# biotite-dev/springcraft

Measured on AMD Instinct MI355X. Metric: ANM modes/sec (Hessian build + full eigensolve), N=2000 C-alpha, higher is better.
Workload: dtype f64; 1 GPU; C3: N=2000 C-alpha ANM, HinsenForceField (no cutoff), full 6000x6000 eigensolve, all modes + vectors; parallelism=independent structures sharded over GPUs, no data-path collective

## Files before the change

### springcraft_amd/csrc/eigh_internal.h

```cpp
#pragma once

#include "common.h"
#include "gemm_f64.h"

struct TriLayout {
  int n, nb;
  long long slab;
  long long vw;
  long long wv;
  long long xraw;
  long long ypart;
  long long dpart;
  long long npart;
  long long wvpart;
  long long d, e, tau;
  long long hscale;
  long long rctl;
  long long rrec;
};
inline size_t tri_resident_bytes(int n) { return sizeof(double) * (8 + (size_t)6 * ((n + 63) / 64 * 64)); }

int mirror_lower_batched(sc_ctx* ctx, double* d_a, long long stride_a, int n, int batch);
int prepare_matrix_batched(sc_ctx* ctx, double* d_a, long long stride_a, int n, int batch, double* d_tri_ws,
                           const TriLayout& L);
int unscale_values_batched(sc_ctx* ctx, double* d_w, long long stride_w, int m, int batch, const double* d_tri_ws,
                           const TriLayout& L);

int tridiag_batched(sc_ctx* ctx, double* d_a, long long stride_a, int n, int batch, double* d_ws,
                    const TriLayout& L, const GemmDesc* d_syr2k_descs, float* ms_symv, float* ms_syr2k);
bool resident_enabled(const sc_ctx* ctx);

struct DcNode {
  int lo, mid, hi;
};

struct DcLayout {
  int n;
  int leaf_max;
  long long slab;
  long long dd, ee;
  long long w0, w1;
  long long z;
  long long dl, zz;
  long long ddef;
  long long lam;
  long long tauv;
  long long zhat;
  long long rot_c, rot_s;
  long long scale;
  long long src;
  long long org;
  long long dest;
  long long rot_a, rot_b;
  long long ktop_src, ktop_k;
  long long kbot_src, kbot_k;
  long long cnt;
};

int stedc_batched(sc_ctx* ctx, int n, int batch, const double* d_tri_ws, const TriLayout& TL,
                  double* d_dc_ws, const DcLayout& DL, double* d_w, long long stride_w,
                  double* d_q_out, double* d_q_tmp, double* d_u, long long stride_q,
                  GemmDesc* d_merge_descs );
size_t dc_slab_doubles(int n, DcLayout* out);
int dc_max_nodes(int n, int leaf_max);

int sturm_bisect_batched(sc_ctx* ctx, int n, int batch, const double* d_tri_ws, const TriLayout& TL,
                         double* d_w, long long stride_w);

struct BtLayout {
  int n, nbt, splits;
  long long slab;
  long long vc;
  long long gram;
  long long t;
  long long g12;
  long long tx;
  long long w1;
  long long w2;
  int splits_g;
};
size_t bt_slab_doubles(int n, BtLayout* out);
int bt_desc_count(int n, int batch);
int backtransform_batched(sc_ctx* ctx, double* d_a, long long stride_a, int n, int batch,
                          const double* d_tri_ws, const TriLayout& TL, double* d_bt_ws,
                          const BtLayout& BL, double* d_z, long long stride_z, int ncols, double* d_vt,
                          GemmDesc* d_descs , int off = 1, int phase = 0);

struct SbLayout {
  int n;
  long long slab;
  long long vw, wv;
  long long xv;
  long long qrpart, qrpiv;
  long long qrpart8;
  long long xsplit;
  int symm_split;
  long long small;
  long long cmat;
  long long small2;
  long long p2;
  long long ab;
  int ngroups;
  long long ndia;
  long long vd;
  long long frag;
  long long tau2;
};
size_t sb_slab_doubles(int n, int batch, SbLayout* out);
int sb_desc_count(int n, int batch);
int sb_band_width();
int sytrd_2stage_batched(sc_ctx* ctx, double* d_a, long long stride_a, int n, int batch, double* d_tri_ws,
                         const TriLayout& TL, double* d_sb_ws, const SbLayout& SL, int* d_dia_off ,
                         GemmDesc* d_descs , float* ms_stage1, float* ms_stage2,
                         double* d_band_copy = nullptr);
int bt2_prepare(sc_ctx* ctx, int n, int batch, double* d_sb_ws, const SbLayout& SL, hipStream_t st);
int bt2_batched(sc_ctx* ctx, int n, int batch, double* d_sb_ws, const SbLayout& SL, const int* d_dia_off, double* d_z,
                long long stride_z, int ncols, float* ms_fused = nullptr);

struct WinCount {
  int il, count, start, pad;
};
size_t stein_workspace_doubles(int n, int m);
int stein_batched(sc_ctx* ctx, int n, int batch, const double* d_tri_ws, const TriLayout& TL, int il, int iu,
                  double* d_w, long long stride_w, double* d_x, long long stride_x, double* d_ws,
                  GemmDesc* d_descs , const WinCount* d_win = nullptr);
int window_count_batched(sc_ctx* ctx, int batch, const double* d_tri_ws, const TriLayout& TL, double vl, double vu, int K,
                         WinCount* d_win, long long* d_count, const RaggedRec* d_own = nullptr);
int window_compact_batched(sc_ctx* ctx, int n, int batch, int K, const WinCount* d_win, double* d_w, double* d_v,
                           double* d_w_copy, double* d_v_copy);

int launch_mode_weights(sc_ctx* ctx, const double* d_w, int64_t nvec, int64_t batch, const sc_mode_selection& sel,
                        int64_t nsel, const int64_t* d_counts, double* d_s, const RaggedView* rv);
int msf_chunk(int64_t nsel);
```

### springcraft_amd/csrc/stedc.hip

```cpp
#include <algorithm>
#include <vector>

#include "eigh_internal.h"

namespace {

constexpr double kEps = 2.220446049250313e-16;

__device__ __forceinline__ int* iptr(double* ws, long long off) { return reinterpret_cast<int*>(ws + off); }
__device__ __forceinline__ const int* iptr(const double* ws, long long off) {
  return reinterpret_cast<const int*>(ws + off);
}

__device__ __forceinline__ double wave_sum_all(double v) {
#pragma unroll
  for (int off = 32; off > 0; off >>= 1) v += __shfl_xor(v, off);
  return v;
}
__device__ __forceinline__ double wave_prod_all(double v) {
#pragma unroll
  for (int off = 32; off > 0; off >>= 1) v *= __shfl_xor(v, off);
  return v;
}
__device__ __forceinline__ double wave_max_all(double v) {
#pragma unroll
  for (int off = 32; off > 0; off >>= 1) v = fmax(v, __shfl_xor(v, off));
  return v;
}

__global__ void k_dc_prepare(const double* __restrict__ tri_all, TriLayout TL, double* __restrict__ dc_all,
                             DcLayout DL, const DcNode* __restrict__ nodes, int n_nodes) {
  __shared__ double red[16];
  const double* tri = tri_all + (size_t)blockIdx.x * TL.slab;
  double* ws = dc_all + (size_t)blockIdx.x * DL.slab;
  const int n = DL.n, tid = threadIdx.x;
  double mx = 0.0;
  for (int i = tid; i < n; i += blockDim.x) {
    mx = fmax(mx, fabs(tri[TL.d + i]));
    if (i < n - 1) mx = fmax(mx, fabs(tri[TL.e + i]));
  }
  mx = wave_max_all(mx);
  if ((tid & 63) == 0) red[tid >> 6] = mx;
  __syncthreads();
  mx = 0.0;
  for (int w = 0; w < (int)(blockDim.x >> 6); ++w) mx = fmax(mx, red[w]);
  const double nrm = (mx > 0.0 && mx == mx) ? mx : 1.0;
  const double inv = 1.0 / nrm;
  for (int i = tid; i < n; i += blockDim.x) {
    const double dv = tri[TL.d + i] * inv;
    const double ev = (i < n - 1) ? tri[TL.e + i] * inv : 0.0;
    ws[DL.dd + i] = fabs(dv) < 1e-150 ? 0.0 : dv;
    ws[DL.ee + i] = fabs(ev) < 1e-150 ? 0.0 : ev;
  }
  if (tid == 0) ws[DL.scale] = nrm;
  __syncthreads();
  for (int g = tid; g < n_nodes; g += blockDim.x) {
    const int mid = nodes[g].mid;
    const double r = fabs(ws[DL.ee + mid - 1]);
    ws[DL.dd + mid - 1] -= r;
    ws[DL.dd + mid] -= r;
  }
}

template <int LEAF>
__global__ __launch_bounds__(64) void k_dc_leaves(double* __restrict__ dc_all, DcLayout DL,
                                                  const DcNode* __restrict__ leaves,
                                                  double* __restrict__ q_all, long long stride_q,
                                                  int* __restrict__ fail_flag) {
  __shared__ double Z[LEAF][LEAF + 1];
  __shared__ double d[LEAF], e[LEAF];
  double* ws = dc_all + (size_t)blockIdx.y * DL.slab;
  double* Q = q_all + (size_t)blockIdx.y * stride_q;
  const int lo = leaves[blockIdx.x].lo, hi = leaves[blockIdx.x].hi;
  const int s = hi - lo, n = DL.n;
  const int lane = threadIdx.x;
  if (lane < s) {
    for (int c = 0; c < s; ++c) Z[lane][c] = (c == lane) ? 1.0 : 0.0;
    d[lane] = ws[DL.dd + lo + lane];
    e[lane] = (lane < s - 1) ? ws[DL.ee + lo + lane] : 0.0;
  }
  __syncthreads();
  for (int l = 0; l < s; ++l) {
    int iter = 0;
    int m;
    do {
      for (m = l; m < s - 1; ++m) {
        const double dd = fabs(d[m]) + fabs(d[m + 1]);
        if (fabs(e[m]) <= kEps * dd) break;
      }
      if (m != l) {
        if (++iter > 80) {
          if (lane == 0) atomicExch(fail_flag, 1);
          break;
        }
        double g = (d[l + 1] - d[l]) / (2.0 * e[l]);
        double r = hypot(g, 1.0);
        g = d[m] - d[l] + e[l] / (g + copysign(r, g));
        double sn = 1.0, cs = 1.0, p = 0.0;
        int i;
        for (i = m - 1; i >= l; --i) {
          double f = sn * e[i];
          const double b = cs * e[i];
          r = hypot(f, g);
          __syncthreads();
          e[i + 1] = r;
          if (r == 0.0) {
            d[i + 1] -= p;
            e[m] = 0.0;
            __syncthreads();
            break;
          }
          sn = f / r;
          cs = g / r;
          g = d[i + 1] - p;
          r = (d[i] - g) * sn + 2.0 * cs * b;
          p = sn * r;
          d[i + 1] = g + p;
          g = cs * r - b;
          if (lane < s) {
            f = Z[lane][i + 1];
            Z[lane][i + 1] = sn * Z[lane][i] + cs * f;
            Z[lane][i] = cs * Z[lane][i] - sn * f;
          }
          __syncthreads();
        }
        if (r == 0.0 && i >= l) continue;
        __syncthreads();
        d[l] -= p;
        e[l] = g;
        e[m] = 0.0;
        __syncthreads();
      }
    } while (m != l);
  }
  __syncthreads();
  for (int a = 0; a < s - 1; ++a) {
    int k = a;
    double best = d[a];
    for (int b = a + 1; b < s; ++b)
      if (d[b] < best) { best = d[b]; k = b; }
    __syncthreads();
    if (k != a) {
      const double tmp = d[a];
      __syncthreads();
      d[k] = tmp;
      d[a] = best;
      if (lane < s) {
        const double t2 = Z[lane][a];
        Z[lane][a] = Z[lane][k];
        Z[lane][k] = t2;
      }
    }
    __syncthreads();
  }
  if (lane < s) {
    ws[DL.w0 + lo + lane] = d[lane];
    for (int c = 0; c < s; ++c) Q[(size_t)(lo + c) * n + lo + lane] = Z[lane][c];
  }
}

__global__ void k_dc_zero_offdiag(const DcNode* __restrict__ nodes, double* __restrict__ q_all,
                                  long long stride_q, int n) {
  const DcNode nd = nodes[blockIdx.y];
  double* Q = q_all + (size_t)blockIdx.z * stride_q;
  const int n1 = nd.mid - nd.lo, n2 = nd.hi - nd.mid;
  const long long total = 2LL * n1 * n2;
  for (long long idx = blockIdx.x * (long long)blockDim.x + threadIdx.x; idx < total;
       idx += (long long)gridDim.x * blockDim.x) {
    if (idx < (long long)n1 * n2) {
      const int r = nd.mid + (int)(idx % n2), c = nd.lo + (int)(idx / n2);
      Q[(size_t)c * n + r] = 0.0;
    } else {
      const long long k = idx - (long long)n1 * n2;
      const int r = nd.lo + (int)(k % n1), c = nd.mid + (int)(k / n1);
      Q[(size_t)c * n + r] = 0.0;
    }
  }
}

__global__ __launch_bounds__(1024) void k_dc_setup(double* __restrict__ dc_all, DcLayout DL,
                                                   const DcNode* __restrict__ nodes, int nodes_in_level,
                                                   const double* __restrict__ q_all, long long stride_q,
                                                   long long w_old_off, GemmDesc* __restrict__ descs,
                                                   int use_lds, double* __restrict__ gscratch,
                                                   long long gscratch_stride) {
  extern __shared__ __attribute__((aligned(16))) double lds[];
  __shared__ double red[16];
  __shared__ double s_tol;
  const int g = blockIdx.x, b = blockIdx.y;
  const DcNode nd = nodes[g];
  double* ws = dc_all + (size_t)b * DL.slab;
  const double* Q = q_all + (size_t)b * stride_q;
  const int n = DL.n, lo = nd.lo, mid = nd.mid, hi = nd.hi;
  const int N = hi - lo, n1 = mid - lo;
  const int tid = threadIdx.x, nthr = blockDim.x;
  const double* wold = ws + w_old_off;

  double* sd;
  double* sz;
  int* scol;
  unsigned char* smix;
  unsigned char* sflag;
  if (use_lds) {
    sd = lds;
    sz = lds + N;
    scol = reinterpret_cast<int*>(lds + 2 * N);
    smix = reinterpret_cast<unsigned char*>(scol + N);
  } else {
    double* base = gscratch + (size_t)b * gscratch_stride + 3LL * lo;
    sd = base;
    sz = base + N;
    scol = reinterpret_cast<int*>(base + 2 * N);
    smix = reinterpret_cast<unsigned char*>(scol + N);
  }
  sflag = smix + N;

  const double rho_raw = ws[DL.ee + mid - 1];
  const double sgn = rho_raw < 0.0 ? -1.0 : 1.0;
  const double rho = 2.0 * fabs(rho_raw);
  const double isq2 = 0.7071067811865475244;

  double zmax = 0.0, dmax = 0.0;
  for (int j = tid; j < N; j += nthr) {
    const int col = lo + j;
    const double zj = (j < n1 ? Q[(size_t)col * n + (mid - 1)] : sgn * Q[(size_t)col * n + mid]) * isq2;
    ws[DL.z + col] = zj;
    zmax = fmax(zmax, fabs(zj));
    dmax = fmax(dmax, fabs(wold[col]));
  }
  zmax = wave_max_all(zmax);
  dmax = wave_max_all(dmax);
  if ((tid & 63) == 0) red[tid >> 6] = fmax(zmax, dmax);
  __syncthreads();
  if (tid == 0) {
    double mx = 0.0;
    for (int w = 0; w < (nthr >> 6); ++w) mx = fmax(mx, red[w]);
    s_tol = 8.0 * kEps * mx;
  }
  __syncthreads();
  for (int j = tid; j < N; j += nthr) {
    const double v = wold[lo + j];
    int rank;
    if (j < n1) {
      int a = 0, c = N - n1;
      while (a < c) {
        const int h = (a + c) >> 1;
        if (wold[mid + h] < v) a = h + 1; else c = h;
      }
      rank = j + a;
    } else {
      int a = 0, c = n1;
      while (a < c) {
        const int h = (a + c) >> 1;
        if (wold[lo + h] <= v) a = h + 1; else c = h;
      }
      rank = (j - n1) + a;
    }
    sd[rank] = v;
    sz[rank] = ws[DL.z + lo + j];
    scol[rank] = lo + j;
    smix[rank] = 0;
  }
  __syncthreads();

  const double tol = s_tol;
  int* src = iptr(ws, DL.src);
  int* rot_a = iptr(ws, DL.rot_a);
  int* rot_b = iptr(ws, DL.rot_b);
  int* cnt = iptr(ws, DL.cnt);
  int* ktop_src = iptr(ws, DL.ktop_src);
  int* ktop_k = iptr(ws, DL.ktop_k);
  int* kbot_src = iptr(ws, DL.kbot_src);
  int* kbot_k = iptr(ws, DL.kbot_k);
  __shared__ int wsum[3][16];
  __shared__ int s_nrot;
  const int L = (N + nthr - 1) / nthr;
  const int j0 = min(tid * L, N), j1 = min(j0 + L, N);

  for (int j = tid; j < N; j += nthr) sflag[j] = !(rho * fabs(sz[j]) > tol) ? 1 : 0;
  if (tid == 0) s_nrot = 0;
  __syncthreads();
  int nseed = 0;
  for (int jj = j0; jj < j1; ++jj) {
    if (sflag[jj] & 1) continue;
    int pj = jj - 1;
    while (pj >= 0 && (sflag[pj] & 1)) --pj;
    if (pj < 0) continue;
    double s = sz[pj], c = sz[jj];
    const double tau = hypot(c, s);
    const double t = sd[jj] - sd[pj];
    c /= tau;
    s /= tau;
    if (fabs(t * c * s) <= tol) { sflag[jj] |= 2; ++nseed; }
  }
  const int any_rot = __syncthreads_or(nseed);
  if (any_rot) {
    int is = nseed;
    for (int off = 1; off < 64; off <<= 1) {
      const int us = __shfl_up(is, off);
      if ((tid & 63) >= off) is += us;
    }
    if ((tid & 63) == 63) wsum[0][tid >> 6] = is;
    __syncthreads();
    int bs = 0, total = 0;
    for (int w = 0; w < (nthr >> 6); ++w) {
      if (w < (tid >> 6)) bs += wsum[0][w];
      total += wsum[0][w];
    }
    int pos = bs + is - nseed;
    for (int jj = j0; jj < j1; ++jj)
      if (sflag[jj] & 2) kbot_k[lo + pos++] = jj;
    __syncthreads();
    if (tid == 0) {
      int nrot = 0, done_upto = -1;
      for (int si = 0; si < total; ++si) {
        int jj = kbot_k[lo + si];
        if (jj <= done_upto) continue;
        int pj = jj - 1;
        while (pj >= 0 && (sflag[pj] & 5)) --pj;
        while (true) {
          double s = sz[pj], c = sz[jj];
          const double tau = hypot(c, s);
          const double t = sd[jj] - sd[pj];
          c /= tau;
          s /= tau;
          done_upto = jj;
          if (!(fabs(t * c * s) <= tol)) break;
          sz[jj] = tau;
          sz[pj] = 0.0;
          rot_a[lo + nrot] = scol[pj];
          rot_b[lo + nrot] = scol[jj];
          ws[DL.rot_c + lo + nrot] = c;
          ws[DL.rot_s + lo + nrot] = s;
          ++nrot;
          if (((scol[pj] < mid) != (scol[jj] < mid)) || smix[pj] || smix[jj]) { smix[jj] = 1; smix[pj] = 1; }
          const double tt = sd[pj] * c * c + sd[jj] * s * s;
          sd[jj] = sd[pj] * s * s + sd[jj] * c * c;
          sd[pj] = tt;
          sflag[pj] |= 4;
          pj = jj;
          ++jj;
          while (jj < N && (sflag[jj] & 1)) ++jj;
          if (jj >= N) break;
        }
      }
      s_nrot = nrot;
    }
    __syncthreads();
  }
  {
    int ns = 0, nt = 0, nb = 0;
    for (int j = j0; j < j1; ++j)
      if (!(sflag[j] & 5)) {
        const bool top = scol[j] < mid;
        ++ns;
        nt += (top || smix[j]) ? 1 : 0;
        nb += (!top || smix[j]) ? 1 : 0;
      }
    int is = ns, it = nt, ib = nb;
    for (int off = 1; off < 64; off <<= 1) {
      const int us = __shfl_up(is, off), ut = __shfl_up(it, off), ub = __shfl_up(ib, off);
      if ((tid & 63) >= off) { is += us; it += ut; ib += ub; }
    }
    __syncthreads();
    if ((tid & 63) == 63) { wsum[0][tid >> 6] = is; wsum[1][tid >> 6] = it; wsum[2][tid >> 6] = ib; }
    __syncthreads();
    int bs = 0, bt = 0, bb = 0, ts = 0, tt = 0, tb = 0;
    for (int w = 0; w < (nthr >> 6); ++w) {
      if (w < (tid >> 6)) { bs += wsum[0][w]; bt += wsum[1][w]; bb += wsum[2][w]; }
      ts += wsum[0][w];
      tt += wsum[1][w];
      tb += wsum[2][w];
    }
    int K = bs + is - ns, K1 = bt + it - nt, K3 = bb + ib - nb;
    int ndef = j0 - K;
    for (int j = j0; j < j1; ++j) {
      if (sflag[j] & 5) {
        ws[DL.ddef + hi - 1 - ndef] = sd[j];
        src[hi - 1 - ndef] = scol[j];
        ++ndef;
      } else {
        ws[DL.dl + lo + K] = sd[j];
        ws[DL.zz + lo + K] = sz[j];
        src[lo + K] = scol[j];
        const bool top = scol[j] < mid;
        if (top || smix[j]) { ktop_src[lo + K1] = scol[j]; ktop_k[lo + K1] = K; ++K1; }
        if (!top || smix[j]) { kbot_src[lo + K3] = scol[j]; kbot_k[lo + K3] = K; ++K3; }
        ++K;
      }
    }
    if (tid == 0) {
      cnt[2 * g] = ts;
      cnt[2 * g + 1] = s_nrot;
      GemmDesc& Dt = descs[((size_t)b * nodes_in_level + g) * 2];
      Dt.n = ts;
      Dt.k = tt;
      GemmDesc& Db = descs[((size_t)b * nodes_in_level + g) * 2 + 1];
      Db.n = ts;
      Db.k = tb;
    }
  }
}

__global__ void k_dc_rotate(double* __restrict__ dc_all, DcLayout DL, const DcNode* __restrict__ nodes,
                            double* __restrict__ q_all, long long stride_q) {
  const int g = blockIdx.y, b = blockIdx.z;
  const DcNode nd = nodes[g];
  double* ws = dc_all + (size_t)b * DL.slab;
  const int nrot = iptr(ws, DL.cnt)[2 * g + 1];
  if (nrot == 0) return;
  double* Q = q_all + (size_t)b * stride_q;
  const int n = DL.n;
  const int row = nd.lo + blockIdx.x * blockDim.x + threadIdx.x;
  if (row >= nd.hi) return;
  const int* rot_a = iptr(ws, DL.rot_a) + nd.lo;
  const int* rot_b = iptr(ws, DL.rot_b) + nd.lo;
  for (int q = 0; q < nrot; ++q) {
    const double c = ws[DL.rot_c + nd.lo + q], s = ws[DL.rot_s + nd.lo + q];
    double* pa = Q + (size_t)rot_a[q] * n + row;
    double* pb = Q + (size_t)rot_b[q] * n + row;
    const double qa = *pa, qb = *pb;
    *pa = c * qa - s * qb;
    *pb = s * qa + c * qb;
  }
}

__global__ __launch_bounds__(1024) void k_dc_secular(double* __restrict__ dc_all, DcLayout DL,
                                                     const DcNode* __restrict__ nodes, int use_lds) {
  extern __shared__ __attribute__((aligned(16))) double lds[];
  const int g = blockIdx.y, b = blockIdx.z;
  const DcNode nd = nodes[g];
  double* ws = dc_all + (size_t)b * DL.slab;
  const int K = iptr(ws, DL.cnt)[2 * g];
  const int waves = blockDim.x >> 6;
  if ((int)blockIdx.x * waves >= K) return;
  const int lo = nd.lo;
  const double* dlg = ws + DL.dl + lo;
  const double* zzg = ws + DL.zz + lo;
  const double* dl;
  const double* z2;
  if (use_lds) {
    double* ldl = lds;
    double* lz2 = lds + K;
    for (int i = threadIdx.x; i < K; i += blockDim.x) {
      ldl[i] = dlg[i];
      const double z = zzg[i];
      lz2[i] = z * z;
    }
    __syncthreads();
    dl = ldl;
    z2 = lz2;
  } else {
    dl = dlg;
    z2 = nullptr;
  }
  const int lane = threadIdx.x & 63;
  const int j = blockIdx.x * waves + (threadIdx.x >> 6);
  if (j >= K) return;
  const double rho = 2.0 * fabs(ws[DL.ee + nd.mid - 1]);
  const double rinv = 1.0 / rho;

  auto fsum2 = [&](double dorg, double tau, double& fp) -> double {
    double s = 0.0, sp = 0.0;
    if (z2) {
      for (int i = lane; i < K; i += 64) {
        const double r = 1.0 / ((dl[i] - dorg) - tau);
        const double zr = z2[i] * r;
        s += zr;
        sp += zr * r;
      }
    } else {
      for (int i = lane; i < K; i += 64) {
        const double z = zzg[i];
        const double r = 1.0 / ((dl[i] - dorg) - tau);
        const double zr = z * z * r;
        s += zr;
        sp += zr * r;
      }
    }
    fp = wave_sum_all(sp);
    return rinv + wave_sum_all(s);
  };
  auto fsum = [&](double dorg, double tau) -> double {
    double fp;
    return fsum2(dorg, tau, fp);
  };

  int org;
  bool positive;
  double t_hi;
  double t_start = 0.0;
  double zj2 = 0.0, zk2 = 0.0;
  if (j == K - 1) {
    org = K - 1;
    positive = true;
    double s2 = 0.0;
    if (z2) { for (int i = lane; i < K; i += 64) s2 += z2[i]; }
    else { for (int i = lane; i < K; i += 64) s2 += zzg[i] * zzg[i]; }
    s2 = wave_sum_all(s2);
    t_hi = rho * s2 * (1.0 + 8.0 * kEps) + 1e-300;
  } else {
    const double gap = dl[j + 1] - dl[j];
    const double half = 0.5 * gap;
    const double fm = fsum(dl[j], half);
    if (fm > 0.0) { org = j; positive = true; } else { org = j + 1; positive = false; }
    t_hi = half;
    {
      zj2 = z2 ? z2[j] : zzg[j] * zzg[j];
      zk2 = z2 ? z2[j + 1] : zzg[j + 1] * zzg[j + 1];
      const double c = fm + (zj2 - zk2) / half;
      double t0;
      if (positive) {
        const double a = c * gap + zj2 + zk2, b = zj2 * gap;
        const double disc = sqrt(fabs(a * a - 4.0 * b * c));
        t0 = a > 0.0 ? 2.0 * b / (a + disc) : (a - disc) / (2.0 * c);
      } else {
        const double a = c * gap - zj2 - zk2, b = zk2 * gap;
        const double disc = sqrt(fabs(a * a + 4.0 * b * c));
        t0 = -(a < 0.0 ? 2.0 * b / (a - disc) : -(a + disc) / (2.0 * c));
      }
      if (t0 == t0 && t0 > 0.0 && t0 < t_hi) t_start = t0;
    }
  }
  const double dorg = dl[org];
  unsigned long long lo_b = 0ull, hi_b = (unsigned long long)__double_as_longlong(t_hi);
  unsigned long long t_b = hi_b - ((hi_b - lo_b) >> 1);
  if (t_start > 0.0) t_b = (unsigned long long)__double_as_longlong(t_start);
  unsigned long long probe_dist = 4ull;
  double t_accept = 0.0;
  for (int it = 0; it < 90 && hi_b - lo_b > 1ull; ++it) {
    const double t = __longlong_as_double((long long)t_b);
    double fp;
    const double f = fsum2(dorg, positive ? t : -t, fp);
    const bool go_up = positive ? (f < 0.0) : (f > 0.0);
    if (go_up) lo_b = t_b; else hi_b = t_b;
    if (hi_b - lo_b <= 1ull) break;
    const unsigned long long mid_b = lo_b + ((hi_b - lo_b) >> 1);
    double tn;
    bool model_step = false;
    if (j < K - 1 && fabs(f) * t < 0.25 * (positive ? zj2 : zk2)) {
      model_step = true;
      const double tau = positive ? t : -t;
      const double dj = (dl[j] - dorg) - tau, dk = (dl[j + 1] - dorg) - tau;
      const double dw = fp;
      double c;
      if (positive) {
        const double q = zj2 / (dj * dj);
        c = f - dk * dw - (dl[j] - dl[j + 1]) * q;
      } else {
        const double q = zk2 / (dk * dk);
        c = f - dj * dw - (dl[j + 1] - dl[j]) * q;
      }
      const double a = (dj + dk) * f - dj * dk * dw;
      const double b = dj * dk * f;
      double eta;
      if (c == 0.0) {
        eta = a != 0.0 ? b / a : -f / dw;
      } else {
        const double disc = sqrt(fabs(a * a - 4.0 * b * c));
        eta = a <= 0.0 ? (a - disc) / (2.0 * c) : 2.0 * b / (a + disc);
      }
      if (f * eta >= 0.0) eta = -f / dw;
      const double tau_n = tau + eta;
      tn = positive ? tau_n : -tau_n;
    } else {
      const double fpt = positive ? fp : -fp;
      const double den = fpt * t + f;
      tn = fpt * t * t / den;
    }
    unsigned long long n_b = mid_b;
    if (tn == tn && tn > 0.0 && tn < 1.7e308) {
      const unsigned long long c_b = (unsigned long long)__double_as_longlong(tn);
      if (c_b > lo_b && c_b < hi_b) {
        n_b = c_b;
        const unsigned long long step = c_b > t_b ? c_b - t_b : t_b - c_b;
#ifndef DC_STRICT_BRACKET
        if (step <= 2ull || (model_step && fabs(tn - t) <= 1e-12 * t)) {
          t_accept = tn;
          break;
        }
#endif
        if (step <= 4ull) {
          const unsigned long long far = go_up ? c_b + probe_dist : (c_b > probe_dist ? c_b - probe_dist : 0ull);
          n_b = (far > lo_b && far < hi_b) ? far : mid_b;
          probe_dist *= 8ull;
        }
      }
    }
    t_b = n_b;
  }
  double t_best = __longlong_as_double((long long)hi_b);
  if (t_accept > 0.0) {
    t_best = t_accept;
  } else if (lo_b > 0ull) {
    const double t_lo = __longlong_as_double((long long)lo_b);
    const double f_lo = fabs(fsum(dorg, positive ? t_lo : -t_lo));
    const double f_hi = fabs(fsum(dorg, positive ? t_best : -t_best));
    if (f_lo < f_hi) t_best = t_lo;
  }
  if (lane == 0) {
    const double tau = positive ? t_best : -t_best;
    iptr(ws, DL.org)[lo + j] = org;
    ws[DL.tauv + lo + j] = tau;
    ws[DL.lam + lo + j] = dorg + tau;
  }
}

__global__ __launch_bounds__(256) void k_dc_zhat(double* __restrict__ dc_all, DcLayout DL,
                                                 const DcNode* __restrict__ nodes) {
  const int g = blockIdx.y, b = blockIdx.z;
  const DcNode nd = nodes[g];
  double* ws = dc_all + (size_t)b * DL.slab;
  const int K = iptr(ws, DL.cnt)[2 * g];
  const int i = blockIdx.x * (blockDim.x >> 6) + (threadIdx.x >> 6);
  if (i >= K) return;
  const int lane = threadIdx.x & 63, lo = nd.lo;
  const double* dl = ws + DL.dl + lo;
  const int* org = iptr(ws, DL.org) + lo;
  const double* tauv = ws + DL.tauv + lo;
  const double di = dl[i];
  double prod = 1.0;
  for (int j = lane; j < K; j += 64) {
    const double num = (di - dl[org[j]]) - tauv[j];
    prod *= (j == i) ? num : num / (di - dl[j]);
  }
  prod = wave_prod_all(prod);
  if (lane == 0) ws[DL.zhat + lo + i] = copysign(sqrt(fabs(prod)), ws[DL.zz + lo + i]);
}

__global__ __launch_bounds__(256) void k_dc_vectors(double* __restrict__ dc_all, DcLayout DL,
                                                    const DcNode* __restrict__ nodes,
                                                    double* __restrict__ u_all, long long stride_u) {
  __shared__ double red[4];
  const int g = blockIdx.y, b = blockIdx.z;
  const DcNode nd = nodes[g];
  double* ws = dc_all + (size_t)b * DL.slab;
  const int K = iptr(ws, DL.cnt)[2 * g];
  const int j = blockIdx.x;
  if (j >= K) return;
  const int lo = nd.lo, n = DL.n;
  const double* dl = ws + DL.dl + lo;
  const double* zh = ws + DL.zhat + lo;
  const double dorg = dl[iptr(ws, DL.org)[lo + j]];
  const double tau = ws[DL.tauv + lo + j];
  double* U = u_all + (size_t)b * stride_u + (size_t)(lo + j) * n + lo;
  double ss = 0.0;
  for (int i = threadIdx.x; i < K; i += blockDim.x) {
    const double u = zh[i] / ((dl[i] - dorg) - tau);
    U[i] = u;
    ss += u * u;
  }
  ss = wave_sum_all(ss);
  if ((threadIdx.x & 63) == 0) red[threadIdx.x >> 6] = ss;
  __syncthreads();
  const double inv = 1.0 / sqrt((red[0] + red[1]) + (red[2] + red[3]));
  for (int i = threadIdx.x; i < K; i += blockDim.x) U[i] *= inv;
}

__global__ __launch_bounds__(256) void k_dc_finalize(double* __restrict__ dc_all, DcLayout DL,
                                                     const DcNode* __restrict__ nodes, long long w_new_off) {
  const int g = blockIdx.y, b = blockIdx.z;
  const DcNode nd = nodes[g];
  double* ws = dc_all + (size_t)b * DL.slab;
  const int K = iptr(ws, DL.cnt)[2 * g];
  const int lo = nd.lo, hi = nd.hi, N = hi - lo, ndef = N - K;
  const int idx = blockIdx.x * blockDim.x + threadIdx.x;
  if (idx >= N) return;
  const double* lam = ws + DL.lam + lo;
  int* dest = iptr(ws, DL.dest);
  double* wnew = ws + w_new_off;
  auto defval = [&](int e) { return ws[DL.ddef + hi - 1 - e]; };
  if (idx < K) {
    const double v = lam[idx];
    int c = 0;
    for (int e = 0; e < ndef; ++e) c += defval(e) < v;
    dest[lo + idx] = lo + idx + c;
    wnew[lo + idx + c] = v;
  } else {
    const int e = idx - K;
    const double v = defval(e);
    int a = 0, c = K;
    while (a < c) {
      const int h = (a + c) >> 1;
      if (lam[h] <= v) a = h + 1; else c = h;
    }
    int r = a;
    for (int f = 0; f < ndef; ++f) {
      const double u = defval(f);
      r += (u < v) || (u == v && f < e);
    }
    dest[lo + idx] = lo + r;
    wnew[lo + r] = v;
  }
}

__global__ __launch_bounds__(256) void k_dc_copy_deflated(double* __restrict__ dc_all, DcLayout DL,
                                                          const DcNode* __restrict__ nodes,
                                                          const double* __restrict__ q_old_all,
                                                          double* __restrict__ q_new_all,
                                                          long long stride_q) {
  const int g = blockIdx.y, b = blockIdx.z;
  const DcNode nd = nodes[g];
  double* ws = dc_all + (size_t)b * DL.slab;
  const int K = iptr(ws, DL.cnt)[2 * g];
  const int lo = nd.lo, hi = nd.hi, N = hi - lo;
  const int e = blockIdx.x;
  if (e >= N - K) return;
  const int n = DL.n;
  const int scol = iptr(ws, DL.src)[hi - 1 - e];
  const int dcol = iptr(ws, DL.dest)[lo + K + e];
  const double* qs = q_old_all + (size_t)b * stride_q + (size_t)scol * n + lo;
  double* qd = q_new_all + (size_t)b * stride_q + (size_t)dcol * n + lo;
  for (int r = threadIdx.x; r < N; r += blockDim.x) qd[r] = qs[r];
}

__global__ void k_dc_unscale(const double* __restrict__ dc_all, DcLayout DL, long long w_off,
                             double* __restrict__ w_out, long long stride_w) {
  const double* ws = dc_all + (size_t)blockIdx.y * DL.slab;
  const int i = blockIdx.x * blockDim.x + threadIdx.x;
  if (i < DL.n) w_out[(size_t)blockIdx.y * stride_w + i] = ws[w_off + i] * ws[DL.scale];
}

struct Tree {
  std::vector<DcNode> leaves;
  std::vector<std::vector<DcNode>> levels;
};

Tree build_tree(int n, int leaf_max) {
  int depth = 0;
  while (((n + (1 << depth) - 1) >> depth) > leaf_max) ++depth;
  std::vector<std::vector<DcNode>> by_depth(depth + 1);
  by_depth[0].push_back(DcNode{0, n / 2, n});
  for (int dlev = 0; dlev < depth; ++dlev) {
    for (const DcNode& nd : by_depth[dlev]) {
      by_depth[dlev + 1].push_back(DcNode{nd.lo, nd.lo + (nd.mid - nd.lo) / 2, nd.mid});
      by_depth[dlev + 1].push_back(DcNode{nd.mid, nd.mid + (nd.hi - nd.mid) / 2, nd.hi});
    }
  }
  Tree t;
  t.leaves = by_depth[depth];
  for (int dlev = depth - 1; dlev >= 0; --dlev) t.levels.push_back(by_depth[dlev]);
  return t;
}

constexpr int kLeafMax = 32;
constexpr int kLdsCapSetup = 7000;
constexpr int kLdsCapSecular = 9800;

}

int dc_max_nodes(int n, int leaf_max) {
  Tree t = build_tree(n, leaf_max);
  size_t total = t.leaves.size();
  for (auto& l : t.levels) total += l.size();
  return (int)total;
}

size_t dc_slab_doubles(int n, DcLayout* out) {
  DcLayout L{};
  L.n = n;
  L.leaf_max = kLeafMax;
  long long off = 0;
  const long long nn = ((long long)n + 7) / 8 * 8;
  auto take = [&](long long cnt) { long long o = off; off += (cnt + 7) / 8 * 8; return o; };
  L.dd = take(nn); L.ee = take(nn); L.w0 = take(nn); L.w1 = take(nn); L.z = take(nn);
  L.dl = take(nn); L.zz = take(nn); L.ddef = take(nn); L.lam = take(nn); L.tauv = take(nn);
  L.zhat = take(nn); L.rot_c = take(nn); L.rot_s = take(nn); L.scale = take(8);
  L.src = take(nn); L.org = take(nn); L.dest = take(nn); L.rot_a = take(nn); L.rot_b = take(nn);
  L.ktop_src = take(nn); L.ktop_k = take(nn); L.kbot_src = take(nn); L.kbot_k = take(nn);
  L.cnt = take(2LL * dc_max_nodes(n, kLeafMax) + 8);
  L.slab = off;
  if (out) *out = L;
  return (size_t)off;
}

__global__ __launch_bounds__(1024) void k_dc_desc_flops(const GemmDesc* __restrict__ d, int count, double* __restrict__ out) {
  __shared__ double part[16];
  double a = 0.0;
  for (int r = threadIdx.x; r < count; r += 1024) a += 2.0 * (double)d[r].m * (double)d[r].n * (double)d[r].k;
#pragma unroll
  for (int off = 32; off > 0; off >>= 1) a += __shfl_xor(a, off);
  if ((threadIdx.x & 63) == 0) part[threadIdx.x >> 6] = a;
  __syncthreads();
  if (threadIdx.x == 0) {
    double t = 0.0;
    for (int w = 0; w < 16; ++w) t += part[w];
    *out = t;
  }
}

int stedc_batched(sc_ctx* ctx, int n, int batch, const double* d_tri_ws, const TriLayout& TL,
                  double* d_dc_ws, const DcLayout& DL, double* d_w, long long stride_w, double* d_q_out,
                  double* d_q_tmp, double* d_u, long long stride_q, GemmDesc* d_merge_descs) {
  hipStream_t st = ctx->stream;
  Tree tree = build_tree(n, kLeafMax);
  const int nlev = (int)tree.levels.size();

  std::vector<DcNode> flat(tree.leaves);
  std::vector<size_t> lev_off(nlev);
  for (int l = 0; l < nlev; ++l) {
    lev_off[l] = flat.size();
    flat.insert(flat.end(), tree.levels[l].begin(), tree.levels[l].end());
  }
  const size_t n_internal = flat.size() - tree.leaves.size();
  const size_t node_bytes = align_up(flat.size() * sizeof(DcNode), 256);
  const size_t big_bytes = n > kLdsCapSetup ? (size_t)batch * 3 * n * sizeof(double) : 0;
  SC_TRY(sc_reserve_dc_aux(ctx, node_bytes + 256 + big_bytes));
  DcNode* d_nodes = reinterpret_cast<DcNode*>(ctx->dc_aux);
  int* d_fail = reinterpret_cast<int*>(ctx->d_status + 1);
  double* d_big = big_bytes ? reinterpret_cast<double*>(reinterpret_cast<char*>(d_nodes) + node_bytes + 256) : nullptr;
  SC_TRY(sc_stage_upload(ctx, d_nodes, flat.data(), flat.size() * sizeof(DcNode)));

  auto qbuf = [&](int stage) { return ((nlev - stage) % 2 == 0) ? d_q_out : d_q_tmp; };

  std::vector<GemmDesc> h_descs;
  std::vector<size_t> desc_off(nlev);
  for (int l = 0; l < nlev; ++l) {
    desc_off[l] = h_descs.size();
    const auto& nodes = tree.levels[l];
    const double* q_old = qbuf(l);
    double* q_new = qbuf(l + 1);
    for (int b = 0; b < batch; ++b)
      for (size_t g = 0; g < nodes.size(); ++g) {
        const DcNode& nd = nodes[g];
        auto ip = [&](long long off) { return reinterpret_cast<const int*>(d_dc_ws + (size_t)b * DL.slab + off) + nd.lo; };
        for (int half = 0; half < 2; ++half) {
          const int r0 = half == 0 ? nd.lo : nd.mid;
          GemmDesc D{};
          D.a = q_old + (size_t)b * stride_q + r0;
          D.sa_i = 1; D.sa_k = n;
          D.a_kidx = ip(half == 0 ? DL.ktop_src : DL.kbot_src);
          D.b = d_u + (size_t)b * stride_q + (size_t)nd.lo * n + nd.lo;
          D.sb_k = 1; D.sb_j = n;
          D.b_kidx = ip(half == 0 ? DL.ktop_k : DL.kbot_k);
          D.c = q_new + (size_t)b * stride_q + r0;
          D.ldc = n;
          D.c_jidx = ip(DL.dest);
          D.m = half == 0 ? nd.mid - nd.lo : nd.hi - nd.mid; D.n = 0; D.k = 0;
          D.alpha = 1.0; D.beta = 0.0;
          h_descs.push_back(D);
        }
      }
  }
  if (!h_descs.empty()) SC_TRY(sc_stage_upload(ctx, d_merge_descs, h_descs.data(), h_descs.size() * sizeof(GemmDesc)));

  hipLaunchKernelGGL(k_dc_prepare, dim3((unsigned)batch), dim3(1024), 0, st, d_tri_ws, TL, d_dc_ws, DL,
                     d_nodes + tree.leaves.size(), (int)n_internal);
  hipLaunchKernelGGL((k_dc_leaves<kLeafMax>), dim3((unsigned)tree.leaves.size(), (unsigned)batch), dim3(64),
                     0, st, d_dc_ws, DL, d_nodes, qbuf(0), stride_q, d_fail);

  PhaseTimer t_gemm(ctx, "dc_gemm", st);
  for (int l = 0; l < nlev; ++l) {
    const auto& nodes = tree.levels[l];
    const int G = (int)nodes.size();
    const DcNode* dn = d_nodes + lev_off[l];
    int maxN = 0;
    for (auto& nd : nodes) maxN = std::max(maxN, nd.hi - nd.lo);
    double* q_old = qbuf(l);
    double* q_new = qbuf(l + 1);
    const long long w_old = (l % 2 == 0) ? DL.w0 : DL.w1;
    const long long w_new = (l % 2 == 0) ? DL.w1 : DL.w0;
    GemmDesc* descs = d_merge_descs + desc_off[l];

    hipLaunchKernelGGL(k_dc_zero_offdiag,
                       dim3((unsigned)std::min(1024, (maxN * maxN / 2 + 255) / 256 + 1), (unsigned)G,
                            (unsigned)batch),
                       dim3(256), 0, st, dn, q_old, stride_q, n);
    {
      const int use_lds = maxN <= kLdsCapSetup ? 1 : 0;
      const size_t lds = use_lds ? (size_t)maxN * 22 + 32 : 0;
      const int threads = maxN >= 1024 ? 1024 : (maxN >= 256 ? 256 : 64);
      hipLaunchKernelGGL(k_dc_setup, dim3((unsigned)G, (unsigned)batch), dim3(threads), lds, st, d_dc_ws, DL,
                         dn, G, q_old, stride_q, w_old, descs, use_lds, d_big, (long long)3 * n);
    }
    hipLaunchKernelGGL(k_dc_rotate, dim3((unsigned)((maxN + 255) / 256), (unsigned)G, (unsigned)batch),
                       dim3(256), 0, st, d_dc_ws, DL, dn, q_old, stride_q);
    {
      const int use_lds = maxN <= kLdsCapSecular ? 1 : 0;
      const int threads = maxN >= 2048 ? 1024 : 256;
      const int waves = threads / 64;
      const size_t lds = use_lds ? (size_t)maxN * 16 + 16 : 0;
      hipLaunchKernelGGL(k_dc_secular, dim3((unsigned)((maxN + waves - 1) / waves), (unsigned)G, (unsigned)batch),
                         dim3(threads), lds, st, d_dc_ws, DL, dn, use_lds);
    }
    hipLaunchKernelGGL(k_dc_zhat, dim3((unsigned)((maxN + 3) / 4), (unsigned)G, (unsigned)batch), dim3(256), 0,
                       st, d_dc_ws, DL, dn);
    hipLaunchKernelGGL(k_dc_vectors, dim3((unsigned)maxN, (unsigned)G, (unsigned)batch), dim3(256), 0, st,
                       d_dc_ws, DL, dn, d_u, stride_q);
    hipLaunchKernelGGL(k_dc_finalize, dim3((unsigned)((maxN + 255) / 256), (unsigned)G, (unsigned)batch),
                       dim3(256), 0, st, d_dc_ws, DL, dn, w_new);
    hipLaunchKernelGGL(k_dc_copy_deflated, dim3((unsigned)maxN, (unsigned)G, (unsigned)batch), dim3(256), 0, st,
                       d_dc_ws, DL, dn, q_old, q_new, stride_q);
    t_gemm.start();
    SC_TRY(launch_gemm_f64(ctx, descs, 2 * G * batch, (maxN + 1) / 2, maxN, kGemmTile, 1, true, false,
                           kGemmAmBk));
    t_gemm.stop();
  }
  const long long w_final = (nlev % 2 == 0) ? DL.w0 : DL.w1;
  hipLaunchKernelGGL(k_dc_unscale, dim3((unsigned)((n + 255) / 256), (unsigned)batch), dim3(256), 0, st,
                     d_dc_ws, DL, w_final, d_w, stride_w);
  SC_HIP(ctx, hipGetLastError());

  t_gemm.finish();
  if (ctx->profiling && !h_descs.empty()) {
    double* d_flops = reinterpret_cast<double*>(reinterpret_cast<char*>(d_nodes) + node_bytes);
    hipLaunchKernelGGL(k_dc_desc_flops, dim3(1), dim3(1024), 0, st, d_merge_descs, (int)h_descs.size(), d_flops);
    double h_flops = 0.0;
    SC_HIP(ctx, hipMemcpyAsync(&h_flops, d_flops, sizeof(double), hipMemcpyDeviceToHost, st));
    SC_HIP(ctx, hipStreamSynchronize(st));
    bool found = false;
    for (auto& ph : ctx->phases)
      if (ph.first == "dc_gemm_gflop") { ph.second = h_flops * 1e-9; found = true; }
    if (!found) ctx->phases.emplace_back("dc_gemm_gflop", h_flops * 1e-9);
  }
  return SC_OK;
}
```

Baseline: 177,900 modes/s.

## Speed up D&C secular kernels with fast reciprocal, LDS staging, and register-held vectors

The secular-equation inner loops swap the IEEE double division for a hardware reciprocal estimate refined by two Newton steps. Each root's shifted origin is stored in a new workspace array, so the zhat and vector kernels read it directly instead of through an indirect org[] lookup. k_dc_zhat stages dl, origin and tau in shared memory in chunks of 1024 for the block's four waves. k_dc_vectors keeps up to 16 computed entries per thread in registers, avoiding a write-then-reread-and-rescale pass over U. The trade-offs are possible last-ulp accuracy differences from the Newton reciprocal, extra register pressure, and more workspace.

```diff
diff --git a/springcraft_amd/csrc/eigh_internal.h b/springcraft_amd/csrc/eigh_internal.h
--- a/springcraft_amd/csrc/eigh_internal.h
+++ b/springcraft_amd/csrc/eigh_internal.h
@@ -45,6 +45,7 @@
   long long ddef;
   long long lam;
   long long tauv;
+  long long dorgv;
   long long zhat;
   long long rot_c, rot_s;
   long long scale;
diff --git a/springcraft_amd/csrc/stedc.hip b/springcraft_amd/csrc/stedc.hip
--- a/springcraft_amd/csrc/stedc.hip
+++ b/springcraft_amd/csrc/stedc.hip
@@ -26,6 +26,13 @@
 #pragma unroll
   for (int off = 32; off > 0; off >>= 1) v = fmax(v, __shfl_xor(v, off));
   return v;
+}
+
+__device__ __forceinline__ double rcp_newton(double x) {
+  const double r0 = __builtin_amdgcn_rcp(x);
+  double r = fma(fma(-x, r0, 1.0), r0, r0);
+  r = fma(fma(-x, r, 1.0), r, r);
+  return fabs(r0) <= 1.7976931348623157e308 ? r : r0;
 }
 
 __global__ void k_dc_prepare(const double* __restrict__ tri_all, TriLayout TL, double* __restrict__ dc_all,
@@ -464,7 +471,7 @@
     double s = 0.0, sp = 0.0;
     if (z2) {
       for (int i = lane; i < K; i += 64) {
-        const double r = 1.0 / ((dl[i] - dorg) - tau);
+        const double r = rcp_newton((dl[i] - dorg) - tau);
         const double zr = z2[i] * r;
         s += zr;
         sp += zr * r;
@@ -472,7 +479,7 @@
     } else {
       for (int i = lane; i < K; i += 64) {
         const double z = zzg[i];
-        const double r = 1.0 / ((dl[i] - dorg) - tau);
+        const double r = rcp_newton((dl[i] - dorg) - tau);
         const double zr = z * z * r;
         s += zr;
         sp += zr * r;
@@ -602,9 +609,12 @@
     const double tau = positive ? t_best : -t_best;
     iptr(ws, DL.org)[lo + j] = org;
     ws[DL.tauv + lo + j] = tau;
+    ws[DL.dorgv + lo + j] = dorg;
     ws[DL.lam + lo + j] = dorg + tau;
   }
 }
+
+constexpr int kZhatChunk = 1024;
 
 __global__ __launch_bounds__(256) void k_dc_zhat(double* __restrict__ dc_all, DcLayout DL,
                                                  const DcNode* __restrict__ nodes) {
@@ -612,21 +622,37 @@
   const DcNode nd = nodes[g];
   double* ws = dc_all + (size_t)b * DL.slab;
   const int K = iptr(ws, DL.cnt)[2 * g];
-  const int i = blockIdx.x * (blockDim.x >> 6) + (threadIdx.x >> 6);
-  if (i >= K) return;
+  if ((int)blockIdx.x * 4 >= K) return;
+  const int i = blockIdx.x * 4 + (threadIdx.x >> 6);
   const int lane = threadIdx.x & 63, lo = nd.lo;
   const double* dl = ws + DL.dl + lo;
-  const int* org = iptr(ws, DL.org) + lo;
+  const double* dorgv = ws + DL.dorgv + lo;
   const double* tauv = ws + DL.tauv + lo;
-  const double di = dl[i];
+  __shared__ double s_dl[kZhatChunk], s_dorg[kZhatChunk], s_tau[kZhatChunk];
+  const double di = i < K ? dl[i] : 0.0;
   double prod = 1.0;
-  for (int j = lane; j < K; j += 64) {
-    const double num = (di - dl[org[j]]) - tauv[j];
-    prod *= (j == i) ? num : num / (di - dl[j]);
-  }
+  for (int j0 = 0; j0 < K; j0 += kZhatChunk) {
+    const int cnt = min(kZhatChunk, K - j0);
+    if (j0 > 0) __syncthreads();
+    for (int t = threadIdx.x; t < cnt; t += 256) {
+      s_dl[t] = dl[j0 + t];
+      s_dorg[t] = dorgv[j0 + t];
+      s_tau[t] = tauv[j0 + t];
+    }
+    __syncthreads();
+    if (i < K) {
+      for (int t = lane; t < cnt; t += 64) {
+        const double num = (di - s_dorg[t]) - s_tau[t];
+        prod *= (j0 + t == i) ? num : num / (di - s_dl[t]);
+      }
+    }
+  }
+  if (i >= K) return;
   prod = wave_prod_all(prod);
   if (lane == 0) ws[DL.zhat + lo + i] = copysign(sqrt(fabs(prod)), ws[DL.zz + lo + i]);
 }
+
+constexpr int kVecKeep = 16;
 
 __global__ __launch_bounds__(256) void k_dc_vectors(double* __restrict__ dc_all, DcLayout DL,
                                                     const DcNode* __restrict__ nodes,
@@ -641,20 +667,31 @@
   const int lo = nd.lo, n = DL.n;
   const double* dl = ws + DL.dl + lo;
   const double* zh = ws + DL.zhat + lo;
-  const double dorg = dl[iptr(ws, DL.org)[lo + j]];
+  const double dorg = ws[DL.dorgv + lo + j];
   const double tau = ws[DL.tauv + lo + j];
   double* U = u_all + (size_t)b * stride_u + (size_t)(lo + j) * n + lo;
+  double keep[kVecKeep];
   double ss = 0.0;
-  for (int i = threadIdx.x; i < K; i += blockDim.x) {
+#pragma unroll
+  for (int r = 0; r < kVecKeep; ++r) {
+    const int i = threadIdx.x + r * 256;
+    keep[r] = i < K ? zh[i] / ((dl[i] - dorg) - tau) : 0.0;
+    ss += keep[r] * keep[r];
+  }
+  for (int i = threadIdx.x + kVecKeep * 256; i < K; i += 256) {
     const double u = zh[i] / ((dl[i] - dorg) - tau);
-    U[i] = u;
     ss += u * u;
   }
   ss = wave_sum_all(ss);
   if ((threadIdx.x & 63) == 0) red[threadIdx.x >> 6] = ss;
   __syncthreads();
   const double inv = 1.0 / sqrt((red[0] + red[1]) + (red[2] + red[3]));
-  for (int i = threadIdx.x; i < K; i += blockDim.x) U[i] *= inv;
+#pragma unroll
+  for (int r = 0; r < kVecKeep; ++r) {
+    const int i = threadIdx.x + r * 256;
+    if (i < K) U[i] = keep[r] * inv;
+  }
+  for (int i = threadIdx.x + kVecKeep * 256; i < K; i += 256) U[i] = zh[i] / ((dl[i] - dorg) - tau) * inv;
 }
 
 __global__ __launch_bounds__(256) void k_dc_finalize(double* __restrict__ dc_all, DcLayout DL,
@@ -764,7 +801,7 @@
   const long long nn = ((long long)n + 7) / 8 * 8;
   auto take = [&](long long cnt) { long long o = off; off += (cnt + 7) / 8 * 8; return o; };
   L.dd = take(nn); L.ee = take(nn); L.w0 = take(nn); L.w1 = take(nn); L.z = take(nn);
-  L.dl = take(nn); L.zz = take(nn); L.ddef = take(nn); L.lam = take(nn); L.tauv = take(nn);
+  L.dl = take(nn); L.zz = take(nn); L.ddef = take(nn); L.lam = take(nn); L.tauv = take(nn); L.dorgv = take(nn);
   L.zhat = take(nn); L.rot_c = take(nn); L.rot_s = take(nn); L.scale = take(8);
   L.src = take(nn); L.org = take(nn); L.dest = take(nn); L.rot_a = take(nn); L.rot_b = take(nn);
   L.ktop_src = take(nn); L.ktop_k = take(nn); L.kbot_src = take(nn); L.kbot_k = take(nn);
```

Result: no change. 178,900 modes/s, median of 6 (+0.5%).
